# taiyaki-go/motioncheck_ccm_slam

Hardware: AMD Instinct MI355X
Metric: ORB extract+match Mfeatures/s and GBA iter/s (2k KF, 200k pts) @1/2/4/8 GPU (higher is better)
Workload: dtype u8; 1 GPU; configs[1]: 256 synthetic 752x480 frames per GPU, 8-level pyramid, 1000 features, FAST+quadtree+rBRIEF, then 1000x1000 brute-force Hamming on the 255 consecutive pairs; frames_per_gpu=256

## Files before the change

motioncheck_ccm_slam_amd/csrc/orb_device.h:

```cpp
#pragma once
#include <hip/hip_runtime.h>
#include "orb_types.h"

#define WAVE 64

typedef unsigned short fc_us2 __attribute__((ext_vector_type(2)));
__device__ __forceinline__ fc_us2 fc_pk(unsigned x) { return __builtin_bit_cast(fc_us2, x); }

__device__ __forceinline__ int lane_id() { return threadIdx.x & 63; }
__device__ __forceinline__ unsigned long long lanemask_lt() { return (1ull << lane_id()) - 1ull; }

__device__ __forceinline__ void xcd_work_item(int on, int& x, int& y)
{
    x = (int)blockIdx.x; y = (int)blockIdx.y;
    if (!on) return;
    const unsigned gx = gridDim.x, total = gx * gridDim.y;
    const unsigned lin = blockIdx.y * gx + blockIdx.x;
    unsigned w;
    if (on == 1) {
        const unsigned xcd = lin & 7u, q = total >> 3, rem = total & 7u;
        w = xcd * q + (xcd < rem ? xcd : rem) + (lin >> 3);
    } else {
        const unsigned C = (unsigned)on, span = 8u * C;
        const unsigned full = total - total % span;
        if (lin >= full) w = lin;
        else {
            const unsigned xcd = lin & 7u, j = lin >> 3;
            const unsigned super = j / C, within = j - super * C;
            w = (super * 8u + xcd) * C + within;
        }
    }
    unsigned q = (unsigned)((float)w * __frcp_rn((float)gx));
    if (q * gx > w) q--; else if ((q + 1u) * gx <= w) q++;
    y = (int)q; x = (int)(w - q * gx);
}

__device__ __forceinline__ int wave_incl_scan(int v)
{
    const int lane = lane_id();
#pragma unroll
    for (int d = 1; d < 64; d <<= 1) {
        int y = __shfl_up(v, d, 64);
        if (lane >= d) v += y;
    }
    return v;
}
__device__ __forceinline__ int wave_sum(int v)
{
#pragma unroll
    for (int d = 32; d >= 1; d >>= 1) v += __shfl_xor(v, d, 64);
    return v;
}
__device__ __forceinline__ void wave_sum2_dpp(int& x, int& y)
{
#define WS2_STEP(ctrl, rows) { const int tx = __builtin_amdgcn_update_dpp(0, x, ctrl, rows, 0xf, false); \
                               const int ty = __builtin_amdgcn_update_dpp(0, y, ctrl, rows, 0xf, false); x += tx; y += ty; }
    WS2_STEP(0xb1, 0xf)
    WS2_STEP(0x4e, 0xf)
    WS2_STEP(0x141, 0xf)
    WS2_STEP(0x140, 0xf)
    WS2_STEP(0x142, 0xa)
    WS2_STEP(0x143, 0xc)
#undef WS2_STEP
    x = __builtin_amdgcn_readlane(x, 63);
    y = __builtin_amdgcn_readlane(y, 63);
}

__host__ __device__ inline int fast_score16(int v, const int* r)
{
    int d[16];
#pragma unroll
    for (int k = 0; k < 16; k++) d[k] = v - r[k];
    int lo3[16], hi3[16];
#pragma unroll
    for (int k = 0; k < 16; k++) {
        const int a = d[k], b = d[(k + 1) & 15], c = d[(k + 2) & 15];
        lo3[k] = min(a, min(b, c));
        hi3[k] = max(a, max(b, c));
    }
    int A = -256, B = 256;
#pragma unroll
    for (int k = 0; k < 16; k++) {
        A = max(A, min(lo3[k], min(lo3[(k + 3) & 15], lo3[(k + 6) & 15])));
        B = min(B, max(hi3[k], max(hi3[(k + 3) & 15], hi3[(k + 6) & 15])));
    }
    return max(A, -B) - 1;
}

__host__ __device__ inline int fast_min3(int a, int b, int c)
{
#if defined(__HIP_DEVICE_COMPILE__)
    int r; asm("v_min3_i32 %0, %1, %2, %3" : "=v"(r) : "v"(a), "v"(b), "v"(c)); return r;
#else
    return std::min(a, std::min(b, c));
#endif
}
__host__ __device__ inline int fast_max3(int a, int b, int c)
{
#if defined(__HIP_DEVICE_COMPILE__)
    int r; asm("v_max3_i32 %0, %1, %2, %3" : "=v"(r) : "v"(a), "v"(b), "v"(c)); return r;
#else
    return std::max(a, std::max(b, c));
#endif
}
__host__ __device__ inline int fast_mad24(int a, int b, int c)
{
#if defined(__HIP_DEVICE_COMPILE__)
    int r; asm("v_mad_i32_i24 %0, %1, %2, %3" : "=v"(r) : "v"(a), "v"(b), "v"(c)); return r;
#else
    return a * b + c;
#endif
}
__host__ __device__ inline int fast_arc16(const int* e)
{
    int w3[16], w9[16];
#pragma unroll
    for (int k = 0; k < 16; k++) w3[k] = fast_min3(e[k], e[(k + 1) & 15], e[(k + 2) & 15]);
#pragma unroll
    for (int k = 0; k < 16; k++) w9[k] = fast_min3(w3[k], w3[(k + 3) & 15], w3[(k + 6) & 15]);
    int m = fast_max3(w9[0], w9[1], w9[2]);
#pragma unroll
    for (int k = 3; k < 15; k += 2) m = fast_max3(m, w9[k], w9[k + 1]);
    return max(m, w9[15]);
}

__host__ __device__ inline int fast_arc16_split(int v, const int* r, int t_lo, bool darker, bool* again)
{
    const int bm = min(max(r[0], r[8]), max(r[4], r[12])), dm = max(min(r[0], r[8]), min(r[4], r[12]));
    const bool can_b = !darker && bm > v + t_lo, can_d = darker || dm < v - t_lo;
    *again = can_b && can_d;
    const int s = can_b ? 1 : -1, c = can_b ? -v : v;
    int e[16];
#pragma unroll
    for (int k = 0; k < 16; k++) e[k] = fast_mad24(s, r[k], c);
    return fast_arc16(e);
}

#define FC_WAVES 4
#define FC_ITEM_STRIDE (64 * FC_WAVES)
struct FcItem { int rr, dw; };
__host__ __device__ inline FcEnum fc_enum(int dw_lo, int dw_hi)
{
    FcEnum e{};
    const int n = dw_hi >= dw_lo ? dw_hi - dw_lo + 1 : 0, d = n > 0 ? n : 1;
    e.n_dw = (short)n; e.d_step = (short)(FC_ITEM_STRIDE % d); e.r_step = (short)(FC_ITEM_STRIDE / d);
    e.nd_inv = (1u << 20) / (unsigned)d + 1u;
    return e;
}
__host__ __device__ inline int fc_item_runs(int bh, int n_dw) { return bh > 6 && n_dw > 0 ? ((bh - 6) * n_dw + 63) >> 6 : 0; }
__host__ __device__ inline FcItem fc_item_start(int dw_lo, int n_dw, unsigned nd_inv, int w, int l)
{
    const int it = 64 * w + l;
    FcItem i;
    i.rr = (int)(((unsigned)it * nd_inv) >> 20);
    i.dw = dw_lo + it - i.rr * n_dw;
    return i;
}
__host__ __device__ inline void fc_item_step(FcItem& i, int dw_end, int n_dw, int d_step, int r_step)
{
    const int d = i.dw + d_step;
    const bool wrap = d >= dw_end;
    i.dw = wrap ? d - n_dw : d;
    i.rr += r_step + (wrap ? 1 : 0);
}
__host__ __device__ inline bool fc_item_valid(const FcItem& i, int bh) { return i.rr < bh - 6; }
__host__ __device__ inline int fc_item_pos0(const FcItem& i, int P)
{
#if defined(__HIP_DEVICE_COMPILE__)
    return __mul24(i.rr, P) + 3 * P + 4 * i.dw;
#else
    return (3 + i.rr) * P + 4 * i.dw;
#endif
}
```

motioncheck_ccm_slam_amd/csrc/orb_octree.hip:

```cpp
#include <hip/hip_runtime.h>
#include "orb_types.h"
#include "orb_device.h"

struct OctNodes {
    int* first; int* count;
    short* x0; short* y0; short* x1; short* y1;
    uint8_t* buf;
};
#define OCT_SET_BYTES 20
#define OCT_NODE_LDS 72

__device__ __forceinline__ OctNodes oct_carve(char* base, int cap)
{
    OctNodes n;
    n.first = reinterpret_cast<int*>(base);              base += 4 * cap;
    n.count = reinterpret_cast<int*>(base);              base += 4 * cap;
    n.x0 = reinterpret_cast<short*>(base);               base += 2 * cap;
    n.y0 = reinterpret_cast<short*>(base);               base += 2 * cap;
    n.x1 = reinterpret_cast<short*>(base);               base += 2 * cap;
    n.y1 = reinterpret_cast<short*>(base);               base += 2 * cap;
    n.buf = reinterpret_cast<uint8_t*>(base);
    return n;
}

__device__ __forceinline__ int key_x(unsigned k) { return (int)(k & 0xFFFu); }
__device__ __forceinline__ int key_y(unsigned k) { return (int)((k >> 12) & 0xFFFu); }

__device__ __forceinline__ void wave_sync_mem()
{
    __threadfence_block();
    __syncthreads();
}

__device__ __forceinline__ int oct_nonempty(const int* cc, int p)
{
    return (cc[4 * p] > 0) + (cc[4 * p + 1] > 0) + (cc[4 * p + 2] > 0) + (cc[4 * p + 3] > 0);
}

#ifdef OCT_STAMPS
__device__ unsigned long long oct_stamps[64];
__device__ int oct_stamp_n;
#define OCT_STAMP() do { if (threadIdx.x == 0 && blockIdx.x == 0 && blockIdx.y == 0) { const int i__ = oct_stamp_n; if (i__ < 64) { oct_stamps[i__] = __builtin_amdgcn_s_memtime(); oct_stamp_n = i__ + 1; } } } while (0)
extern "C" int ccm_debug_oct_stamps(unsigned long long* out, int* n)
{
    if (hipMemcpyFromSymbol(n, HIP_SYMBOL(oct_stamp_n), 4, 0, hipMemcpyDeviceToHost) != hipSuccess) return -1;
    const int zero = 0;
    if (hipMemcpyFromSymbol(out, HIP_SYMBOL(oct_stamps), 64 * 8, 0, hipMemcpyDeviceToHost) != hipSuccess) return -1;
    return hipMemcpyToSymbol(HIP_SYMBOL(oct_stamp_n), &zero, 4, 0, hipMemcpyHostToDevice) == hipSuccess ? 0 : -1;
}
#else
#define OCT_STAMP() do { } while (0)
#endif
#ifndef OCT_LDS_KEYS
#define OCT_LDS_KEYS 2048
#endif
#ifndef OCT_WAVES
#define OCT_WAVES 4
#endif
#ifndef OCT_WPE
#define OCT_WPE 5
#endif
#define OCT_OCC __attribute__((amdgpu_waves_per_eu(OCT_WPE, OCT_WPE)))
__global__ __launch_bounds__(64 * OCT_WAVES) OCT_OCC void k_octree(const OrbGeom g, const OrbCell* __restrict__ cells,
                                               const unsigned* __restrict__ slots, const int* __restrict__ cell_count,
                                               unsigned* keysA, unsigned* keysB,
                                               unsigned* __restrict__ out, int* __restrict__ out_count,
                                               int* __restrict__ status, int reg_keys_on)
{
    extern __shared__ __attribute__((aligned(16))) char smem[];
    OCT_STAMP();
    const int level = blockIdx.y, f = blockIdx.x + g.frame0, lane = lane_id(), wv = threadIdx.x >> 6;
    const OrbLevel& L = g.lv[level];
    const int cap = g.list_cap;
    OctNodes cur = oct_carve(smem, cap);
    OctNodes nxt = oct_carve(smem + (size_t)cap * OCT_SET_BYTES, cap);
    int* cc = reinterpret_cast<int*>(smem + (size_t)cap * 2 * OCT_SET_BYTES);
    int* ord = cc + 4 * cap;
    int* cbase = ord + cap;
    int* mark = cbase + cap;
    int* gain = mark + cap;
    int* shared_len = gain + cap;

    unsigned* kb[2] = { keysA + (long long)f * g.keys_per_frame + L.key_first,
                        keysB + (long long)f * g.keys_per_frame + L.key_first };
    unsigned* lkeys = reinterpret_cast<unsigned*>(shared_len + 4);
    unsigned* best = lkeys + OCT_LDS_KEYS;
    unsigned short* surv_pos = reinterpret_cast<unsigned short*>(best + cap);
    const int N = L.quota;
    int* ocount = out_count + (long long)f * g.nlevels + level;

    const int* ccount = cell_count + (long long)f * g.ncells + L.cell_first;
    const unsigned* fslots = slots + (long long)f * g.slots_per_frame;
    int total = 0;
    for (int base = 0; base < L.ncells; base += 64 * OCT_WAVES) {
        int cnt[OCT_WAVES];
#pragma unroll
        for (int u = 0; u < OCT_WAVES; u++) {
            const int ci = base + 64 * u + lane;
            cnt[u] = ci < L.ncells ? ccount[ci] : 0;
        }
        const int myci = base + 64 * wv + lane;
        const int sfirst = myci < L.ncells ? cells[L.cell_first + myci].slot_first : 0;
        int mydst = 0, mycnt = 0;
#pragma unroll
        for (int u = 0; u < OCT_WAVES; u++) {
            const int incl = wave_incl_scan(cnt[u]);
            if (u == wv) { mydst = total + incl - cnt[u]; mycnt = cnt[u]; }
            total += __shfl(incl, 63, 64);
        }
        OCT_STAMP();
        const unsigned* sp = fslots + sfirst;
        for (int k = 0; k < mycnt; k += 8) {
            unsigned v[8];
#pragma unroll
            for (int u = 0; u < 8; u++) v[u] = sp[min(k + u, mycnt - 1)];
#pragma unroll
            for (int u = 0; u < 8; u++)
                if (k + u < mycnt && mydst + k + u < L.key_cap) {
                    kb[0][mydst + k + u] = v[u];
                    if (mydst + k + u < OCT_LDS_KEYS) lkeys[mydst + k + u] = v[u];
                }
        }
    }
    OCT_STAMP();
    if (total > L.key_cap) { if (lane == 0) atomicOr(status, 1); total = L.key_cap; }
    const int n = total;
    if (n == 0 || N <= 0) { if (threadIdx.x == 0) *ocount = 0; return; }
    const bool small = reg_keys_on && n <= OCT_LDS_KEYS;
    wave_sync_mem();
    OCT_STAMP();

    const int tid = threadIdx.x;
    const int R = L.roots;
    constexpr int OCT_KPT = OCT_LDS_KEYS / (64 * OCT_WAVES);
    unsigned mykey[OCT_KPT]; int mynode[OCT_KPT];
#pragma unroll
    for (int j = 0; j < OCT_KPT; j++) { mykey[j] = 0u; mynode[j] = 0; }
    if (small) {
#pragma unroll
        for (int j = 0; j < OCT_KPT; j++) { const int k = tid + 64 * OCT_WAVES * j; if (k < n) mykey[j] = lkeys[k]; }
    }
    auto for_keys = [&](auto&& fn, int mode) {
        if (small) {
#pragma unroll
            for (int j = 0; j < OCT_KPT; j++) { const int k = tid + 64 * OCT_WAVES * j; if (k < n) fn(mykey[j], mynode[j], k); }
        } else {
            for (int k = tid; k < n; k += 64 * OCT_WAVES) {
                const unsigned key = kb[0][k];
                int node = mode == 2 ? 0 : (int)kb[1][k];
                fn(key, node, k);
                if (mode != 0) kb[1][k] = (unsigned)node;
            }
        }
    };
    if (tid < ORB_MAX_ROOTS) cc[tid] = 0;
    __syncthreads();
    for_keys([&](unsigned key, int& node, int) {
        int r = (int)((float)key_x(key) / L.hx); r = min(r, R - 1);
        node = r;
        atomicAdd(&cc[r], 1);
    }, 2);
    __syncthreads();
    if (tid == 0) {
        int p = 0;
        for (int r = 0; r < R; r++) {
            gain[r] = p;
            if (cc[r] == 0) continue;
            cur.x0[p] = (short)(int)(L.hx * (float)r);
            cur.x1[p] = (short)(int)(L.hx * (float)(r + 1));
            cur.y0[p] = 0; cur.y1[p] = (short)L.bh;
            cur.count[p] = cc[r];
            p++;
        }
        *shared_len = p;
    }
    __syncthreads();
    for_keys([&](unsigned, int& node, int) { node = gain[node]; }, 1);
    wave_sync_mem();
    int len = *shared_len;

    OCT_STAMP();
    bool finish = false, careful = false;
    int guard = 0;
    const unsigned long long lt = lanemask_lt();
    while (!finish) {
        if (++guard > 512) { if (lane == 0) atomicOr(status, 2); break; }
        const int prev = len;
        int nc = 0;
        for (int base = 0; base < len; base += 64) {
            const int p = base + lane;
            const bool dv = p < len && cur.count[p] > 1;
            const unsigned long long m = __ballot(dv);
            if (dv) ord[nc + __popcll(m & lt)] = p;
            nc += __popcll(m);
        }
        for (int i = tid; i < 4 * len; i += 64 * OCT_WAVES) cc[i] = 0;
        __syncthreads();
        for_keys([&](unsigned key, int& node, int) {
            const int p = node;
            if (cur.count[p] > 1) {
                const int csx = cur.x0[p] + (cur.x1[p] - cur.x0[p] + 1) / 2, csy = cur.y0[p] + (cur.y1[p] - cur.y0[p] + 1) / 2;
                atomicAdd(&cc[4 * p + (key_x(key) < csx ? 0 : 1) + (key_y(key) < csy ? 0 : 2)], 1);
            }
        }, 0);
        wave_sync_mem();
        OCT_STAMP();
        int nd = nc;
        if (careful) {
            const int m_c = nc;
            for (int base = 64 * wv; base < len; base += 64 * OCT_WAVES) {
                const int p = base + lane;
                const int myc = p < len ? cur.count[p] : 0;
                if (myc > 1) {
                    int rank = 0;
                    for (int q0 = 0; q0 < len; q0 += 8) {
                        int cq[8];
#pragma unroll
                        for (int u = 0; u < 8; u++) cq[u] = cur.count[min(q0 + u, len - 1)];
#pragma unroll
                        for (int u = 0; u < 8; u++) {
                            const int q = q0 + u;
                            rank += (q < len && cq[u] > 1 && (cq[u] > myc || (cq[u] == myc && q < p))) ? 1 : 0;
                        }
                    }
                    ord[rank] = p;
                    gain[rank] = oct_nonempty(cc, p) - 1;
                }
            }
            wave_sync_mem();
            int run = len, K = m_c - 1;
            bool found = false;
            for (int base = 0; base < m_c && !found; base += 64) {
                const int k = base + lane;
                const int gn = k < m_c ? gain[k] : 0;
                const int incl = wave_incl_scan(gn);
                const unsigned long long hit = __ballot(k < m_c && run + incl >= N);
                if (hit != 0ull) { K = base + __ffsll((long long)hit) - 1; found = true; }
                run += __shfl(incl, 63, 64);
            }
            nd = m_c > 0 ? K + 1 : 0;
        }
        OCT_STAMP();
        int T = 0;
        for (int base = 0; base < nd; base += 64) {
            const int k = base + lane;
            const int ne = k < nd ? oct_nonempty(cc, ord[k]) : 0;
            const int incl = wave_incl_scan(ne);
            if (k < nd) cbase[k] = T + incl - ne;
            T += __shfl(incl, 63, 64);
        }
        for (int base = 0; base < len; base += 64) { const int p = base + lane; if (p < len) mark[p] = 0; }
        __builtin_amdgcn_s_waitcnt(0xc07f);
        __builtin_amdgcn_wave_barrier();
        for (int base = 0; base < nd; base += 64) { const int k = base + lane; if (k < nd) mark[ord[k]] = k + 1; }
        wave_sync_mem();
        int nsurv = 0;
        for (int base = 0; base < len; base += 64) {
            const int p = base + lane;
            const bool sv = p < len && mark[p] == 0;
            const unsigned long long m = __ballot(sv);
            if (sv) {
                const int dest = T + nsurv + __popcll(m & lt);
                if (dest < cap) {
                    nxt.x0[dest] = cur.x0[p]; nxt.y0[dest] = cur.y0[p]; nxt.x1[dest] = cur.x1[p]; nxt.y1[dest] = cur.y1[p];
                    nxt.count[dest] = cur.count[p];
                    surv_pos[p] = (unsigned short)dest;
                }
            }
            nsurv += __popcll(m);
        }
        const int newlen = T + nsurv;
        if (newlen > cap) { if (lane == 0) atomicOr(status, 4); break; }
        int newExpand = 0;
        for (int base = 0; base < nd; base += 64) {
            const int k = base + lane;
            int gt1 = 0;
            if (k < nd) {
                const int p = ord[k];
                const int px0 = cur.x0[p], py0 = cur.y0[p], px1 = cur.x1[p], py1 = cur.y1[p];
                const int sx = px0 + (px1 - px0 + 1) / 2, sy = py0 + (py1 - py0 + 1) / 2;
                int ci = cbase[k];
#pragma unroll
                for (int q = 0; q < 4; q++) {
                    const int c = cc[4 * p + q];
                    if (c > 0) {
                        const int dest = T - 1 - ci;
                        nxt.x0[dest] = (short)((q & 1) ? sx : px0);
                        nxt.x1[dest] = (short)((q & 1) ? px1 : sx);
                        nxt.y0[dest] = (short)((q & 2) ? sy : py0);
                        nxt.y1[dest] = (short)((q & 2) ? py1 : sy);
                        nxt.count[dest] = c;
                        ci++;
                        gt1 += (c > 1);
                    }
                }
            }
            newExpand += wave_sum(gt1);
        }
        wave_sync_mem();
        for_keys([&](unsigned key, int& node, int) {
            const int p = node;
            const int mk = mark[p];
            if (mk == 0) node = surv_pos[p];
            else {
                const int csx = cur.x0[p] + (cur.x1[p] - cur.x0[p] + 1) / 2, csy = cur.y0[p] + (cur.y1[p] - cur.y0[p] + 1) / 2;
                const int q = (key_x(key) < csx ? 0 : 1) + (key_y(key) < csy ? 0 : 2);
                int ci = cbase[mk - 1];
                if (q > 0) ci += cc[4 * p] > 0;
                if (q > 1) ci += cc[4 * p + 1] > 0;
                if (q > 2) ci += cc[4 * p + 2] > 0;
                node = T - 1 - ci;
            }
        }, 1);
        __syncthreads();
        { OctNodes t = cur; cur = nxt; nxt = t; }
        len = newlen;
        OCT_STAMP();
        if (len >= N || len == prev) finish = true;
        else if (!careful && len + 3 * newExpand > N) careful = true;
    }

    unsigned* o = out + (long long)f * g.out_per_frame + L.out_first;
    for (int p = tid; p < len; p += 64 * OCT_WAVES) best[p] = 0u;
    __syncthreads();
    for_keys([&](unsigned key, int& node, int k) { atomicMax(&best[node], (key & 0xFF000000u) | (0xFFFFFFu - (unsigned)k)); }, 0);
    __syncthreads();
    for (int p = tid; p < len && p < L.out_cap; p += 64 * OCT_WAVES) {
        const unsigned kidx = 0xFFFFFFu - (best[p] & 0xFFFFFFu);
        o[p] = small ? lkeys[kidx] : kb[0][kidx];
    }
    if (tid == 0) *ocount = min(len, L.out_cap);
    OCT_STAMP();
}

size_t orb_octree_lds_bytes(int list_cap) { return (size_t)list_cap * OCT_NODE_LDS + 64 + 4 * (size_t)OCT_LDS_KEYS + 8 * (size_t)list_cap; }
void orb_launch_octree(hipStream_t s, const OrbGeom& g_dev, const OrbCell* cells, int nlevels, int nframes, int list_cap,
                       const unsigned* slots, const int* cell_count, unsigned* keysA, unsigned* keysB,
                       unsigned* out, int* out_count, int* status)
{
    static const int key_parallel = !(getenv("CCM_OCT_REG_KEYS") && atoi(getenv("CCM_OCT_REG_KEYS")) == 0);
    hipLaunchKernelGGL(k_octree, dim3(nframes, nlevels), dim3(64 * OCT_WAVES), orb_octree_lds_bytes(list_cap), s,
                       g_dev, cells, slots, cell_count, keysA, keysB, out, out_count, status, key_parallel);
}
```

Before: 321.2 Mfeatures/s.

## Use DPP wave scans, gather octree keys by binary search, pack-rank careful split

```diff
diff --git a/motioncheck_ccm_slam_amd/csrc/orb_device.h b/motioncheck_ccm_slam_amd/csrc/orb_device.h
--- a/motioncheck_ccm_slam_amd/csrc/orb_device.h
+++ b/motioncheck_ccm_slam_amd/csrc/orb_device.h
@@ -37,19 +37,28 @@
 
 __device__ __forceinline__ int wave_incl_scan(int v)
 {
-    const int lane = lane_id();
-#pragma unroll
-    for (int d = 1; d < 64; d <<= 1) {
-        int y = __shfl_up(v, d, 64);
-        if (lane >= d) v += y;
-    }
+#define WSC_STEP(ctrl, rows) v += __builtin_amdgcn_update_dpp(0, v, ctrl, rows, 0xf, false);
+    WSC_STEP(0x111, 0xf)
+    WSC_STEP(0x112, 0xf)
+    WSC_STEP(0x114, 0xf)
+    WSC_STEP(0x118, 0xf)
+    WSC_STEP(0x142, 0xa)
+    WSC_STEP(0x143, 0xc)
+#undef WSC_STEP
     return v;
 }
+__device__ __forceinline__ int wave_last(int incl) { return __builtin_amdgcn_readlane(incl, 63); }
 __device__ __forceinline__ int wave_sum(int v)
 {
-#pragma unroll
-    for (int d = 32; d >= 1; d >>= 1) v += __shfl_xor(v, d, 64);
-    return v;
+#define WS1_STEP(ctrl, rows) v += __builtin_amdgcn_update_dpp(0, v, ctrl, rows, 0xf, false);
+    WS1_STEP(0xb1, 0xf)
+    WS1_STEP(0x4e, 0xf)
+    WS1_STEP(0x141, 0xf)
+    WS1_STEP(0x140, 0xf)
+    WS1_STEP(0x142, 0xa)
+    WS1_STEP(0x143, 0xc)
+#undef WS1_STEP
+    return __builtin_amdgcn_readlane(v, 63);
 }
 __device__ __forceinline__ void wave_sum2_dpp(int& x, int& y)
 {
diff --git a/motioncheck_ccm_slam_amd/csrc/orb_octree.hip b/motioncheck_ccm_slam_amd/csrc/orb_octree.hip
--- a/motioncheck_ccm_slam_amd/csrc/orb_octree.hip
+++ b/motioncheck_ccm_slam_amd/csrc/orb_octree.hip
@@ -23,6 +23,8 @@
     return n;
 }
 
+template <int V> struct OctInt { static constexpr int value = V; };
+
 __device__ __forceinline__ int key_x(unsigned k) { return (int)(k & 0xFFFu); }
 __device__ __forceinline__ int key_y(unsigned k) { return (int)((k >> 12) & 0xFFFu); }
 
@@ -53,6 +55,9 @@
 #endif
 #ifndef OCT_LDS_KEYS
 #define OCT_LDS_KEYS 2048
+#endif
+#ifndef OCT_GATHER_CELLS
+#define OCT_GATHER_CELLS 512
 #endif
 #ifndef OCT_WAVES
 #define OCT_WAVES 4
@@ -91,8 +96,48 @@
 
     const int* ccount = cell_count + (long long)f * g.ncells + L.cell_first;
     const unsigned* fslots = slots + (long long)f * g.slots_per_frame;
+    const int tid = threadIdx.x;
+    const int R = L.roots;
+    constexpr int OCT_KPT = OCT_LDS_KEYS / (64 * OCT_WAVES);
+    unsigned mykey[OCT_KPT]; int mynode[OCT_KPT];
+#pragma unroll
+    for (int j = 0; j < OCT_KPT; j++) { mykey[j] = 0u; mynode[j] = 0; }
+    if (tid < ORB_MAX_ROOTS) cc[tid] = 0;
+    constexpr int OCT_GCH = OCT_GATHER_CELLS / 64, OCT_GPW = OCT_GCH / OCT_WAVES;
+    static_assert(OCT_GCH % OCT_WAVES == 0 && OCT_GPW >= 1, "every wave leaves the offsets of OCT_GPW chunks");
+    int* goffs = reinterpret_cast<int*>(smem);
+    int* gdelta = goffs + 5 * cap;
     int total = 0;
-    for (int base = 0; base < L.ncells; base += 64 * OCT_WAVES) {
+    bool gathered = false;
+    if (reg_keys_on && L.ncells <= min(OCT_GATHER_CELLS, 5 * cap)) {
+        int cnt[OCT_GCH], sf[OCT_GPW], myoff[OCT_GPW];
+#pragma unroll
+        for (int u = 0; u < OCT_GCH; u++) {
+            const int ci = 64 * u + lane;
+            cnt[u] = ci < L.ncells ? ccount[ci] : 0;
+        }
+#pragma unroll
+        for (int v = 0; v < OCT_GPW; v++) {
+            const int ci = 64 * (wv + OCT_WAVES * v) + lane;
+            sf[v] = ci < L.ncells ? cells[L.cell_first + ci].slot_first : 0;
+            myoff[v] = 0;
+        }
+#pragma unroll
+        for (int u = 0; u < OCT_GCH; u++) {
+            const int incl = wave_incl_scan(cnt[u]);
+            if (u % OCT_WAVES == wv) myoff[u / OCT_WAVES] = total + incl - cnt[u];
+            total += wave_last(incl);
+        }
+        if (total <= OCT_LDS_KEYS) {
+#pragma unroll
+            for (int v = 0; v < OCT_GPW; v++) {
+                const int ci = 64 * (wv + OCT_WAVES * v) + lane;
+                if (ci < L.ncells) { goffs[ci] = myoff[v]; gdelta[ci] = sf[v] - myoff[v]; }
+            }
+            gathered = true;
+        } else total = 0;
+    }
+    for (int base = 0; base < L.ncells && !gathered; base += 64 * OCT_WAVES) {
         int cnt[OCT_WAVES];
 #pragma unroll
         for (int u = 0; u < OCT_WAVES; u++) {
@@ -106,9 +151,8 @@
         for (int u = 0; u < OCT_WAVES; u++) {
             const int incl = wave_incl_scan(cnt[u]);
             if (u == wv) { mydst = total + incl - cnt[u]; mycnt = cnt[u]; }
-            total += __shfl(incl, 63, 64);
-        }
-        OCT_STAMP();
+            total += wave_last(incl);
+        }
         const unsigned* sp = fslots + sfirst;
         for (int k = 0; k < mycnt; k += 8) {
             unsigned v[8];
@@ -130,16 +174,6 @@
     wave_sync_mem();
     OCT_STAMP();
 
-    const int tid = threadIdx.x;
-    const int R = L.roots;
-    constexpr int OCT_KPT = OCT_LDS_KEYS / (64 * OCT_WAVES);
-    unsigned mykey[OCT_KPT]; int mynode[OCT_KPT];
-#pragma unroll
-    for (int j = 0; j < OCT_KPT; j++) { mykey[j] = 0u; mynode[j] = 0; }
-    if (small) {
-#pragma unroll
-        for (int j = 0; j < OCT_KPT; j++) { const int k = tid + 64 * OCT_WAVES * j; if (k < n) mykey[j] = lkeys[k]; }
-    }
     auto for_keys = [&](auto&& fn, int mode) {
         if (small) {
 #pragma unroll
@@ -153,31 +187,60 @@
             }
         }
     };
-    if (tid < ORB_MAX_ROOTS) cc[tid] = 0;
-    __syncthreads();
-    for_keys([&](unsigned key, int& node, int) {
+    auto count_root = [&](unsigned key, int& node, int) {
         int r = (int)((float)key_x(key) / L.hx); r = min(r, R - 1);
         node = r;
         atomicAdd(&cc[r], 1);
-    }, 2);
-    __syncthreads();
-    if (tid == 0) {
-        int p = 0;
-        for (int r = 0; r < R; r++) {
-            gain[r] = p;
-            if (cc[r] == 0) continue;
-            cur.x0[p] = (short)(int)(L.hx * (float)r);
-            cur.x1[p] = (short)(int)(L.hx * (float)(r + 1));
-            cur.y0[p] = 0; cur.y1[p] = (short)L.bh;
-            cur.count[p] = cc[r];
-            p++;
-        }
-        *shared_len = p;
-    }
-    __syncthreads();
-    for_keys([&](unsigned, int& node, int) { node = gain[node]; }, 1);
+    };
+    if (gathered) {
+        auto fetch = [&](auto nj) {
+            constexpr int NJ = decltype(nj)::value;
+            int pos[NJ];
+#pragma unroll
+            for (int j = 0; j < NJ; j++) pos[j] = 0;
+#pragma unroll
+            for (int step = OCT_GATHER_CELLS / 2; step >= 1; step >>= 1) {
+#pragma unroll
+                for (int j = 0; j < NJ; j++) {
+                    const int k = tid + 64 * OCT_WAVES * j, t = pos[j] + step;
+                    const int first = goffs[min(t, L.ncells - 1)];
+                    pos[j] = (t < L.ncells && first <= k) ? t : pos[j];
+                }
+            }
+#pragma unroll
+            for (int j = 0; j < NJ; j++) pos[j] = gdelta[pos[j]];
+#pragma unroll
+            for (int j = 0; j < NJ; j++) { const int k = tid + 64 * OCT_WAVES * j; if (k < n) mykey[j] = fslots[k + pos[j]]; }
+#pragma unroll
+            for (int j = 0; j < NJ; j++) {
+                const int k = tid + 64 * OCT_WAVES * j;
+                if (k < n) { lkeys[k] = mykey[j]; count_root(mykey[j], mynode[j], k); }
+            }
+        };
+        if (n <= 64 * OCT_WAVES * (OCT_KPT / 2)) fetch(OctInt<OCT_KPT / 2>()); else fetch(OctInt<OCT_KPT>());
+    } else {
+        if (small) {
+#pragma unroll
+            for (int j = 0; j < OCT_KPT; j++) { const int k = tid + 64 * OCT_WAVES * j; if (k < n) mykey[j] = lkeys[k]; }
+        }
+        for_keys(count_root, 2);
+    }
     wave_sync_mem();
-    int len = *shared_len;
+    OCT_STAMP();
+    unsigned rpos = 0u;
+    int len = 0;
+#pragma unroll
+    for (int r = 0; r < ORB_MAX_ROOTS; r++)
+        if (r < R) { rpos |= (unsigned)len << (4 * r); len += cc[r] > 0; }
+    if (tid < R && cc[tid] > 0) {
+        const int p = (int)((rpos >> (4 * tid)) & 15u);
+        cur.x0[p] = (short)(int)(L.hx * (float)tid);
+        cur.x1[p] = (short)(int)(L.hx * (float)(tid + 1));
+        cur.y0[p] = 0; cur.y1[p] = (short)L.bh;
+        cur.count[p] = cc[tid];
+    }
+    for_keys([&](unsigned, int& node, int) { node = (int)((rpos >> (4 * node)) & 15u); }, 1);
+    wave_sync_mem();
 
     OCT_STAMP();
     bool finish = false, careful = false;
@@ -208,7 +271,39 @@
         int nd = nc;
         if (careful) {
             const int m_c = nc;
-            for (int base = 64 * wv; base < len; base += 64 * OCT_WAVES) {
+            const bool packed = n < (1 << 15);
+            if (packed) {
+                unsigned* pk = best;
+                const int len16 = (len + 15) & ~15;
+                for (int base = 0; base < len16; base += 64) {
+                    const int p = base + lane;
+                    if (p < len16) {
+                        const int c = p < len ? cur.count[p] : 0;
+                        pk[p] = c > 1 ? ((unsigned)c << 16) | (0xFFFFu - (unsigned)p) : 0u;
+                    }
+                }
+                __builtin_amdgcn_s_waitcnt(0xc07f);
+                __builtin_amdgcn_wave_barrier();
+                const uint4* pk4 = reinterpret_cast<const uint4*>(pk);
+                for (int base = 64 * wv; base < len; base += 64 * OCT_WAVES) {
+                    const int p = base + lane;
+                    const unsigned mine = p < len ? pk[p] : 0u;
+                    if (mine != 0u) {
+                        int rank = 0;
+                        for (int q0 = 0; q0 < len16; q0 += 16) {
+                            uint4 a[4];
+#pragma unroll
+                            for (int u = 0; u < 4; u++) a[u] = pk4[(q0 >> 2) + u];
+#pragma unroll
+                            for (int u = 0; u < 4; u++)
+                                rank += (a[u].x > mine) + (a[u].y > mine) + (a[u].z > mine) + (a[u].w > mine);
+                        }
+                        ord[rank] = p;
+                        gain[rank] = oct_nonempty(cc, p) - 1;
+                    }
+                }
+            }
+            for (int base = 64 * wv; base < len && !packed; base += 64 * OCT_WAVES) {
                 const int p = base + lane;
                 const int myc = p < len ? cur.count[p] : 0;
                 if (myc > 1) {
@@ -236,7 +331,7 @@
                 const int incl = wave_incl_scan(gn);
                 const unsigned long long hit = __ballot(k < m_c && run + incl >= N);
                 if (hit != 0ull) { K = base + __ffsll((long long)hit) - 1; found = true; }
-                run += __shfl(incl, 63, 64);
+                run += wave_last(incl);
             }
             nd = m_c > 0 ? K + 1 : 0;
         }
@@ -247,7 +342,7 @@
             const int ne = k < nd ? oct_nonempty(cc, ord[k]) : 0;
             const int incl = wave_incl_scan(ne);
             if (k < nd) cbase[k] = T + incl - ne;
-            T += __shfl(incl, 63, 64);
+            T += wave_last(incl);
         }
         for (int base = 0; base < len; base += 64) { const int p = base + lane; if (p < len) mark[p] = 0; }
         __builtin_amdgcn_s_waitcnt(0xc07f);
```

Result: faster. 327.1 Mfeatures/s, median of 6 (+1.8%).
